# nju-websoft/MultiKE

Measured on AMD Instinct MI355X. Metric: scored triples/sec (pos+neg), higher is better.
Workload: dtype f32; 1 GPU; relation-view train step, C2-synth |E|=200000 |R|=550 dim=75 neg=25 batch=5000; n_ent=200000, n_rel=550, dim=75, neg=25, batch=5000, steps_per_epoch=184

## Files before the change

### include/multike_hip.h

```cpp
#ifndef MULTIKE_HIP_H
#define MULTIKE_HIP_H

#include <stdint.h>

#ifdef __cplusplus
extern "C" {
#endif

#define MKE_VERSION 106

#define MKE_OK 0
#define MKE_E_NULL (-1)
#define MKE_E_SHAPE (-2)
#define MKE_E_UNSUPPORTED (-3)
#define MKE_E_RANGE (-4)

#define MKE_LOSS_PARTIALS 2048

#define MKE_MAX_STRIDE 320

#define MKE_OPT_ADAGRAD 0
#define MKE_OPT_SGD 1
#define MKE_OPT_ADAM 2
#define MKE_OPT_ADADELTA 3

int mke_version(void);
const char* mke_last_error(void);

#define MKE_TUNE_DEFAULT (-2)
typedef struct mke_tuning {
  int score_splits, score_half_groups, score_offsets32, score_lane_ids, count_in_score, update_chunk, oc_score_quarter,
      attr_fused_bwd, sampler_fast;
  int reserved[7];
} mke_tuning;
int mke_tuning_init(mke_tuning* t);

int mke_set_option(const char* name, int value, int* old_value);


int mke_triple_score_fwd_bwd(
    const float* ent_table, int64_t n_ent, int ent_normalize,
    const float* rel_table, int64_t n_rel, int rel_normalize,
    int stride, int dim,
    const int32_t* pos_h, const int32_t* pos_r, const int32_t* pos_t, const float* pos_w ,
    int64_t n_pos,
    const int32_t* neg_h, const int32_t* neg_r, const int32_t* neg_t, const float* neg_w ,
    int64_t n_neg, int neg_per_pos,
    float scale,
    float* grad_ent , float* grad_rel , int grad_rel_copies,
    int32_t* touched_ent, int32_t* touched_rel, int32_t tag,
    double* loss_partials ,
    void* stream);

int mke_triple_score_fwd_bwd_det(
    float* ent_table, int64_t n_ent, int ent_normalize, const float* rel_table, int64_t n_rel, int rel_normalize,
    int stride, int dim, const int32_t* pos_h, const int32_t* pos_r, const int32_t* pos_t, const float* pos_w,
    int64_t n_pos, const int32_t* neg_h, const int32_t* neg_r, const int32_t* neg_t, const float* neg_w, int64_t n_neg,
    int neg_per_pos, float scale, float* grad_ent, float* grad_rel, int32_t* touched_ent, int32_t* touched_rel, int32_t tag,
    int32_t* ref_count , float* ent_acc, int optimizer, float lr, float* stage_rows, int64_t* stage_keys,
    int64_t stage_slots, double* loss_partials, void* stream);
int mke_stage_reduce(const float* stage_rows, const int64_t* sorted_keys, const int64_t* order, int64_t n_slots, int stride,
                     float* grad_ent, float* grad_rel, int32_t* touched_ent, int32_t* touched_rel, int32_t tag, void* stream);
int mke_count_entity_refs(const int32_t* pos_h, const int32_t* pos_t, int64_t n_pos, const int32_t* neg_h,
                          const int32_t* neg_t, int64_t n_neg, int neg_per_pos, int32_t* ref_count, void* stream);
int mke_triple_score_fwd_bwd_x(
    float* ent_table, int64_t n_ent, int ent_normalize,
    const float* rel_table, int64_t n_rel, int rel_normalize,
    int stride, int dim,
    const int32_t* pos_h, const int32_t* pos_r, const int32_t* pos_t, const float* pos_w , int64_t n_pos,
    const int32_t* neg_h, const int32_t* neg_r, const int32_t* neg_t, const float* neg_w , int64_t n_neg,
    int neg_per_pos, float scale,
    float* grad_ent, float* grad_rel, int grad_rel_copies,
    int32_t* touched_ent, int32_t* touched_rel, int32_t tag,
    int32_t* ref_count, float* ent_acc , int optimizer, float lr,
    double* loss_partials, void* stream);

struct mke_count_job;
typedef struct mke_hot_rows {
  const int32_t* slot;
  int32_t n_hot, copies;
  int64_t row0;
} mke_hot_rows;
int mke_triple_score_fwd_bwd_xc(
    float* ent_table, int64_t n_ent, int ent_normalize,
    const float* rel_table, int64_t n_rel, int rel_normalize,
    int stride, int dim,
// ... 454 lines not shown
```

### multike_amd/_lib.py

```python
from __future__ import annotations

import ctypes as C
import os

import numpy as np
import torch

_HERE = os.path.dirname(os.path.abspath(__file__))
SO_PATH = os.path.join(_HERE, "libmultike_hip.so")

LOSS_PARTIALS = 2048
MAX_STRIDE = 320
OPT_ADAGRAD, OPT_SGD, OPT_ADAM, OPT_ADADELTA = 0, 1, 2, 3
DENSE_OPTS = {"Adam": OPT_ADAM, "Adadelta": OPT_ADADELTA}
_SUPPORTED_FPL = (1, 2, 3, 4, 5, 6, 7, 8, 10, 12, 13, 16, 20)

SYMBOLS = (
    "mke_version", "mke_last_error", "mke_set_option", "mke_triple_score_fwd_bwd", "mke_triple_score_fwd_bwd_x",
    "mke_count_entity_refs", "mke_triple_score_fwd_bwd_xc", "mke_triple_score_fwd_bwd_xch", "mke_triple_score_fwd_bwd_det", "mke_stage_reduce", "mke_rows_update", "mke_rows_update_multi", "mke_rows_update_multi_count",
    "mke_neg_sample", "mke_tripleset_build", "mke_tripleset_query", "mke_gathered_logistic_fwd_bwd",
    "mke_gathered_alignment_fwd_bwd", "mke_align_fwd_bwd", "mke_gather_rows", "mke_relation_steps",
    "mke_rowset_build", "mke_rowset_remap", "mke_rows_gather_padded", "mke_rows_scatter_add",
    "mke_attr_conv_fwd", "mke_attr_conv_bwd", "mke_attr_tail_z", "mke_attr_tail_loss", "mke_attr_tail_bwd",
    "mke_dense_update", "mke_align_rank", "mke_gemm_f32", "mke_attr_scratch_floats", "mke_attr_step", "mke_attr_steps", "mke_attr_step_phases",
# ... 26 lines not shown
class AlignTableStruct(C.Structure):
    _fields_ = [("table", C.c_void_p), ("acc", C.c_void_p), ("grad", C.c_void_p), ("touched", C.c_void_p), ("n_rows", C.c_int64),
                ("normalize", C.c_int)]


class AlignTermStruct(C.Structure):
    _fields_ = [("a", C.c_int), ("b", C.c_int), ("weight", C.c_float)]


class AlignPlanStruct(C.Structure):
    _fields_ = [("tables", AlignTableStruct * 4), ("n_tables", C.c_int), ("terms", AlignTermStruct * 4), ("n_terms", C.c_int),
                ("stride", C.c_int), ("dim", C.c_int), ("ia", C.c_void_p), ("ib", C.c_void_p),
                ("step_off", C.POINTER(C.c_int64)), ("n_steps", C.c_int), ("optimizer", C.c_int), ("lr", C.c_float),
                ("tag_base", C.c_int32), ("loss_partials", C.c_void_p)]


class MappingViewStruct(C.Structure):
    _fields_ = [("table", C.c_void_p), ("normalize", C.c_int)]


class MappingStepArgs(C.Structure):
    _fields_ = [("ent_table", C.c_void_p), ("n_ent", C.c_int64), ("ent_normalize", C.c_int), ("ent_acc", C.c_void_p),
                ("ent_grad", C.c_void_p), ("ent_touched", C.c_void_p), ("views", MappingViewStruct * 3), ("n_views", C.c_int),
                ("stride", C.c_int), ("dim", C.c_int), ("idx", C.c_void_p), ("n", C.c_int64), ("M", C.c_void_p), ("gM", C.c_void_p),
                ("accM", C.c_void_p), ("orthogonal_weight", C.c_float), ("norm_w", C.c_float), ("scratch", C.c_void_p),
                ("partials", C.c_void_p), ("optimizer", C.c_int), ("lr", C.c_float), ("tag", C.c_int32), ("update", C.c_int)]


class HotRowsStruct(C.Structure):
    _fields_ = [("slot", C.c_void_p), ("n_hot", C.c_int32), ("copies", C.c_int32), ("row0", C.c_int64)]


class OcStepStruct(C.Structure):
    _fields_ = [("ent", C.c_void_p), ("ent_acc", C.c_void_p), ("ent_grad", C.c_void_p), ("ent_touched", C.c_void_p),
                ("ref_count", C.c_void_p), ("n_local", C.c_int64),
                ("rel", C.c_void_p), ("rel_acc", C.c_void_p), ("rel_grad", C.c_void_p), ("rel_grad_copies", C.c_int), ("rel_touched", C.c_void_p),
                ("n_rel", C.c_int64), ("stride", C.c_int), ("dim", C.c_int), ("rank", C.c_int), ("n_ranks", C.c_int),
                ("pos_h", C.c_void_p), ("pos_r", C.c_void_p), ("pos_t", C.c_void_p), ("n_pos", C.c_int64), ("per", C.c_int64),
                ("slot_h", C.c_void_p), ("slot_t", C.c_void_p), ("own_h", C.c_void_p), ("n_own_h", C.c_int64),
                ("own_t", C.c_void_p), ("n_own_t", C.c_int64), ("neg_per_pos", C.c_int), ("capacity", C.c_int64),
                ("codes", C.c_void_p), ("code_off", C.c_int64 * 16),
                ("optimizer", C.c_int), ("lr", C.c_float), ("scale", C.c_float), ("tag", C.c_int32),
                ("n_peers", C.c_int), ("peer_v", C.c_void_p * 16), ("peer_g", C.c_void_p * 16), ("pos_w", C.c_void_p),
                ("hot", HotRowsStruct),
                ("em_coef", C.c_void_p), ("em_pos0", C.c_int64), ("em_refs", C.c_void_p), ("em_rows", C.c_void_p), ("em_off", C.c_void_p),
                ("em_n_rows", C.c_int64), ("em_chunks", C.c_int), ("em_block_floats", C.c_int64), ("em_v", C.c_void_p * 4),
                ("em_gv", C.c_void_p * 4),
                ("em_part", C.c_void_p), ("em_long_rows", C.c_void_p), ("em_long_part0", C.c_void_p), ("em_n_long", C.c_int64),
                ("em_part0", C.c_int64), ("em_partials", C.c_void_p), ("em_mode", C.c_int), ("tuning", C.c_void_p)]


TUNE_DEFAULT = -2
TUNING_FIELDS = ("score_splits", "score_half_groups", "score_offsets32", "score_lane_ids", "count_in_score", "update_chunk",
                 "oc_score_quarter", "attr_fused_bwd", "sampler_fast")


class TuningStruct(C.Structure):
    _fields_ = [(f, C.c_int) for f in TUNING_FIELDS] + [("reserved", C.c_int * 7)]


def tuning(**knobs) -> TuningStruct:
    t = TuningStruct()
    _check(lib().mke_tuning_init(C.byref(t)), "mke_tuning_init")
    for k, v in knobs.items():
        if k not in TUNING_FIELDS:
            raise MultiKEHipError(f"unknown tuning knob {k!r}")
        setattr(t, k, int(v))
    return t


def tuning_ptr(t) -> int | None:
    return C.addressof(t) if t is not None else None


OC_EM_MAX_CHUNKS = 4
OC_EM_WAVES = 32768


class OcEmPlanArgs(C.Structure):
    _fields_ = [("pos_h", C.c_void_p), ("pos_r", C.c_void_p), ("pos_t", C.c_void_p), ("codes", C.c_void_p), ("neg_per_pos", C.c_int),
                ("slot_h", C.c_void_p), ("slot_t", C.c_void_p), ("step_lo", C.c_void_p), ("n_steps", C.c_int), ("chunks", C.c_int),
                ("n_all", C.c_int64), ("max_step", C.c_int64), ("n_ranks", C.c_int), ("rank", C.c_int), ("n_local", C.c_int64), ("n_rel", C.c_int64),
                ("keys", C.c_void_p), ("keys_alt", C.c_void_p), ("capacity", C.c_int64), ("vals_alt", C.c_void_p), ("scratch8", C.c_void_p), ("wave_scratch", C.c_void_p),
                ("refs", C.c_void_p), ("rows", C.c_void_p), ("off", C.c_void_p), ("flags", C.c_void_p), ("scan", C.c_void_p),
                ("step_row0", C.c_void_p), ("n_refs", C.c_void_p),
                ("item_row", C.c_void_p), ("item_off", C.c_void_p), ("item_part", C.c_void_p), ("long_row", C.c_void_p), ("long_part0", C.c_void_p),
                ("step_item0", C.c_void_p), ("step_long0", C.c_void_p), ("step_part0", C.c_void_p),
                ("temp", C.c_void_p), ("temp_bytes", C.c_int64)]


OC_COMM_NCCL, OC_COMM_CALLBACK, OC_COMM_LOOPBACK = 0, 1, 2
OC_CB_MOVE = C.CFUNCTYPE(C.c_int, C.c_void_p, C.c_void_p, C.c_void_p, C.c_int64, C.c_void_p)
OC_CB_REDUCE = C.CFUNCTYPE(C.c_int, C.c_void_p, C.c_void_p, C.c_int64, C.c_void_p)


class OcCommStruct(C.Structure):
    _fields_ = [("kind", C.c_int), ("ctx", C.c_void_p), ("all_gather", C.c_void_p), ("reduce_scatter", C.c_void_p), ("all_reduce", C.c_void_p),
                ("world", C.c_int), ("rank", C.c_int), ("wire_gbps", C.c_float), ("latency_us", C.c_float)]


class OcLoopStruct(C.Structure):
    _fields_ = [("parts", C.c_void_p), ("step_part0", C.c_void_p), ("n_steps", C.c_int), ("chunks", C.c_int),
                ("send", C.c_void_p * 4), ("v_all", C.c_void_p * 4), ("g_all", C.c_void_p * 4), ("gv", C.c_void_p * 4), ("block_floats", C.c_int64),
                ("loss_ring", C.c_void_p), ("loss_stride", C.c_int64), ("tag_base", C.c_int32), ("comm", C.c_void_p), ("comm_stream", C.c_void_p),
                ("overlap_rs", C.c_int)]


class AEPlanStruct(C.Structure):
    _fields_ = [("n_layers", C.c_int), ("dims", C.c_int * 5), ("act", C.c_int), ("normalize", C.c_int),
                ("params", C.c_void_p), ("grads", C.c_void_p), ("acc", C.c_void_p), ("n_params", C.c_int64),
                ("w_off", C.c_int64 * 8), ("b_off", C.c_int64 * 8), ("optimizer", C.c_int), ("lr", C.c_float),
# ... 852 lines not shown
```

### multike_amd/csrc/mke_api.hip

```cpp
#include <cstdarg>
#include <cstdio>
#include <cstring>

#include "mke_common.h"

namespace mke {

static thread_local char g_err[512] = "";

void set_error(const char* fmt, ...) {
  va_list ap;
  va_start(ap, fmt);
  vsnprintf(g_err, sizeof(g_err), fmt, ap);
  va_end(ap);
}

int check_launch(const char* what) {
  const hipError_t e = hipGetLastError();
  if (e != hipSuccess) {
    set_error("%s: launch failed: %s", what, hipGetErrorString(e));
    return (int)e;
  }
  return MKE_OK;
}

}

namespace mke {
int g_score_splits = 0;
int g_score_half_max = -1;
int g_score_o32 = 1;
int g_count_in_score = 1;
int g_score_lane_ids = 1;
int g_update_chunk = 0;
int g_deterministic = 0;
int g_sampler_fast = 1;
int g_attr_fused_bwd = 1;
int g_oc_em_keys64 = 0;
int g_oc_score_quarter = -1;
thread_local const mke_tuning* tl_tuning = nullptr;
}

extern "C" int mke_tuning_init(mke_tuning* t) {
  if (!t) { mke::set_error("mke_tuning_init: NULL"); return MKE_E_NULL; }
  int* f = reinterpret_cast<int*>(t);
  for (size_t i = 0; i < sizeof(mke_tuning) / sizeof(int); ++i) f[i] = MKE_TUNE_DEFAULT;
  return MKE_OK;
}

extern "C" int mke_set_option(const char* name, int value, int* old_value) {
  if (!name) { mke::set_error("mke_set_option: NULL name"); return MKE_E_NULL; }
  if (!strcmp(name, "score_splits")) {
    if (old_value) *old_value = mke::g_score_splits;
    mke::g_score_splits = value < 0 ? 0 : value;
    return MKE_OK;
  }
  if (!strcmp(name, "score_half_groups")) {
    if (old_value) *old_value = mke::g_score_half_max;
    mke::g_score_half_max = value < 0 ? -1 : (value > 64 ? 64 : value);
    return MKE_OK;
  }
  if (!strcmp(name, "score_offsets32")) {
    if (old_value) *old_value = mke::g_score_o32;
    mke::g_score_o32 = value != 0;
    return MKE_OK;
  }
  if (!strcmp(name, "count_in_score")) {
    if (old_value) *old_value = mke::g_count_in_score;
    mke::g_count_in_score = value != 0;
    return MKE_OK;
  }
  if (!strcmp(name, "score_lane_ids")) {
    if (old_value) *old_value = mke::g_score_lane_ids;
    mke::g_score_lane_ids = value != 0;
    return MKE_OK;
  }
  if (!strcmp(name, "update_chunk")) {
    if (old_value) *old_value = mke::g_update_chunk;
    mke::g_update_chunk = value == 16 ? 16 : (value == 64 ? 64 : 0);
    return MKE_OK;
  }
  if (!strcmp(name, "oc_score_quarter")) {
    if (old_value) *old_value = mke::g_oc_score_quarter;
    mke::g_oc_score_quarter = value < 0 ? -1 : (value != 0);
    return MKE_OK;
  }
  if (!strcmp(name, "attr_fused_bwd")) {
    if (old_value) *old_value = mke::g_attr_fused_bwd;
    mke::g_attr_fused_bwd = value != 0;
    return MKE_OK;
  }
  if (!strcmp(name, "sampler_fast")) {
    if (old_value) *old_value = mke::g_sampler_fast;
    mke::g_sampler_fast = value != 0;
    return MKE_OK;
  }
  if (!strcmp(name, "oc_em_keys64")) {
    if (old_value) *old_value = mke::g_oc_em_keys64;
    mke::g_oc_em_keys64 = value != 0;
    return MKE_OK;
  }
  if (!strcmp(name, "deterministic")) {
    if (old_value) *old_value = mke::g_deterministic;
    mke::g_deterministic = value != 0;
    return MKE_OK;
  }
  mke::set_error("mke_set_option: unknown option '%s'", name);
  return MKE_E_UNSUPPORTED;
}

extern "C" int mke_version(void) { return MKE_VERSION; }
extern "C" const char* mke_last_error(void) { return mke::g_err; }
```

### multike_amd/csrc/mke_common.h

```cpp
#pragma once
#include <hip/hip_runtime.h>
#include <stdint.h>

#include "../../include/multike_hip.h"

#define MKE_BLOCK 256
#define MKE_SUBS_PER_BLOCK (MKE_BLOCK / 16)
#define MKE_L2_EPS 1e-12f

namespace mke {

void set_error(const char* fmt, ...);
int check_launch(const char* what);

template <int CTRL>
__device__ __forceinline__ float dpp_mov(float v) {
  return __builtin_bit_cast(
      float, __builtin_amdgcn_update_dpp(0, __builtin_bit_cast(int, v), CTRL, 0xF, 0xF, true));
}

__device__ __forceinline__ float sub16_sum(float v) {
  v += dpp_mov<0xB1>(v);
  v += dpp_mov<0x4E>(v);
  v += dpp_mov<0x141>(v);
// ... 25 lines not shown
__device__ __forceinline__ void atomic_add_f32(float* p, float v) {
  __hip_atomic_fetch_add(p, v, __ATOMIC_RELAXED, __HIP_MEMORY_SCOPE_AGENT);
}

template <int FPL>
__device__ __forceinline__ void atomic_add_row(float* __restrict__ grad, int64_t row, int stride, int dim,
                                               int j, const float (&v)[FPL], float sgn) {
  float* p = grad + row * (int64_t)stride + j;
#pragma unroll
  for (int k = 0; k < FPL; ++k) {
    if (k * 16 + 16 <= dim || k * 16 + j < dim) atomic_add_f32(p + k * 16, sgn * v[k]);
  }
}

__device__ __forceinline__ float softplus_f(float x) {
  return fmaxf(x, 0.f) + __logf(1.0f + __expf(-fabsf(x)));
}
__device__ __forceinline__ float sigmoid_f(float x) { return __builtin_amdgcn_rcpf(1.0f + __expf(-x)); }
__device__ __forceinline__ float tanh_f(float x) {
  const float e = __expf(-2.0f * fabsf(x));
  return copysignf((1.0f - e) * __builtin_amdgcn_rcpf(1.0f + e), x);
}
__device__ __forceinline__ float adagrad_scale(float a) { return __builtin_amdgcn_rsqf(a); }

__device__ __forceinline__ void count_refs_range(const mke_count_job& c, int64_t block, int64_t n_blocks) {
  const int64_t total = c.n_pos + c.n_neg;
  for (int64_t i = block * MKE_BLOCK + threadIdx.x; i < total; i += n_blocks * MKE_BLOCK) {
    if (i < c.n_pos) {
      atomicAdd(&c.ref_count[c.pos_h[i]], 1);
      atomicAdd(&c.ref_count[c.pos_t[i]], 1);
    } else {
      const int64_t n = i - c.n_pos;
      const int64_t g = n / c.neg_per_pos;
      const int a = c.neg_h[n], b = c.neg_t[n];
      if (a != c.pos_h[g]) atomicAdd(&c.ref_count[a], 1);
      if (b != c.pos_t[g]) atomicAdd(&c.ref_count[b], 1);
    }
  }
}

extern thread_local int64_t g_update_touched_hint;
struct UpdateTouchedHint {
  explicit UpdateTouchedHint(int64_t rows) { g_update_touched_hint = rows; }
  ~UpdateTouchedHint() { g_update_touched_hint = 0; }
};

extern thread_local const mke_tuning* tl_tuning;
struct TuningScope {
  const mke_tuning* prev;
  explicit TuningScope(const mke_tuning* t) : prev(tl_tuning) { if (t) tl_tuning = t; }
  ~TuningScope() { tl_tuning = prev; }
};
extern int g_score_splits, g_score_half_max, g_score_o32, g_score_lane_ids, g_count_in_score, g_update_chunk, g_oc_score_quarter,
    g_attr_fused_bwd, g_sampler_fast;
#define MKE_TUNE(field, dflt) ((mke::tl_tuning && mke::tl_tuning->field != MKE_TUNE_DEFAULT) ? mke::tl_tuning->field : (dflt))
inline int tune_score_splits() { const int v = MKE_TUNE(score_splits, g_score_splits); return v < 0 ? 0 : v; }
inline int tune_score_half_max() { const int v = MKE_TUNE(score_half_groups, g_score_half_max); return v < 0 ? -1 : (v > 64 ? 64 : v); }
inline int tune_score_o32() { return MKE_TUNE(score_offsets32, g_score_o32) != 0; }
inline int tune_score_lane_ids() { return MKE_TUNE(score_lane_ids, g_score_lane_ids) != 0; }
inline int tune_count_in_score() { return MKE_TUNE(count_in_score, g_count_in_score) != 0; }
inline int tune_update_chunk() { const int v = MKE_TUNE(update_chunk, g_update_chunk); return v == 16 ? 16 : (v == 64 ? 64 : 0); }
inline int tune_oc_score_quarter() { const int v = MKE_TUNE(oc_score_quarter, g_oc_score_quarter); return v < 0 ? -1 : (v != 0); }
inline int tune_attr_fused_bwd() { return MKE_TUNE(attr_fused_bwd, g_attr_fused_bwd) != 0; }
inline int tune_sampler_fast() { return MKE_TUNE(sampler_fast, g_sampler_fast) != 0; }

__device__ __forceinline__ double block_sum_double(float v) {
  __shared__ double s_part[MKE_BLOCK / 64];
  double d = (double)v;
#pragma unroll
  for (int off = 32; off > 0; off >>= 1) d += __shfl_down(d, off, 64);
  const int wave = threadIdx.x >> 6;
  if ((threadIdx.x & 63) == 0) s_part[wave] = d;
  __syncthreads();
  double tot = 0.0;
  if (threadIdx.x == 0) {
#pragma unroll
    for (int w = 0; w < MKE_BLOCK / 64; ++w) tot += s_part[w];
  }
  return tot;
}

struct DenseJob {
  float* w;
  float* acc;
  float* g;
  int64_t n;
  int optimizer;
  float lr;
  float* ws;
  int ws_n, ws_stride, ws_copies;
};
__device__ __forceinline__ void dense_update_range(const DenseJob& j, int64_t block, int64_t n_blocks) {
  for (int64_t i = block * MKE_BLOCK + threadIdx.x; i < j.n; i += n_blocks * MKE_BLOCK) {
    float gv = j.g[i];
    if (j.ws && i < j.ws_n) {
#pragma unroll 8
      for (int c = 0; c < j.ws_copies; ++c) gv += j.ws[(size_t)c * j.ws_stride + i];
      for (int c = 0; c < j.ws_copies; ++c) j.ws[(size_t)c * j.ws_stride + i] = 0.f;
    }
    j.g[i] = 0.f;
    if (j.optimizer == MKE_OPT_ADAGRAD) {
      const float a = fmaf(gv, gv, j.acc[i]);
      j.acc[i] = a;
      j.w[i] -= j.lr * gv * adagrad_scale(a);
    } else {
      j.w[i] -= j.lr * gv;
    }
  }
}

struct Philox4 {
  uint32_t v[4];
};
__host__ __device__ __forceinline__ Philox4 philox4x32_10(uint32_t c0, uint32_t c1, uint32_t c2, uint32_t c3,
                                                          uint32_t k0, uint32_t k1) {
  const uint32_t M0 = 0xD2511F53u, M1 = 0xCD9E8D57u, W0 = 0x9E3779B9u, W1 = 0xBB67AE85u;
#pragma unroll
// ... 48 lines not shown
```

### multike_amd/csrc/mke_score.hip

```cpp
#include "mke_common.h"

namespace mke {

#ifndef MKE_SCORE_U
#define MKE_SCORE_U 2
#endif

struct ScoreParams {
  const float* ent;
  const float* __restrict__ rel;
  int ent_norm, rel_norm;
  int stride, dim;
  const int32_t* __restrict__ ph;
  const int32_t* __restrict__ pr;
  const int32_t* __restrict__ pt;
  const float* __restrict__ pw;
  int64_t n_pos;
  const int32_t* __restrict__ nh;
  const int32_t* __restrict__ nr;
  const int32_t* __restrict__ nt;
  const float* __restrict__ nw;
  int64_t n_neg;
  int npp;
  int splits;
  float scale;
  float* __restrict__ gent;
  float* __restrict__ grel;
  int grel_copies;
  int64_t grel_copy_elems;
  int32_t* __restrict__ tent;
  int32_t* __restrict__ trel;
  int32_t tag;
  double* __restrict__ lossp;
  int32_t* __restrict__ refcount;
  float* ent_w;
  float* __restrict__ ent_acc;
  int optimizer;
  float lr;
  float* __restrict__ stage_rows;
  int64_t* __restrict__ stage_keys;
  mke_count_job cj;
  int count_blocks;
  const int32_t* __restrict__ hot_slot;
  int32_t n_hot, hot_copies;
  int32_t hot_row0;
};

#define MKE_STAGE_REL (1ll << 40)
__device__ __forceinline__ int64_t stage_slot(int64_t g, int npp, int n, int c) { return ((g * (npp + 1) + n) * 3 + c); }

template <int FPL, bool O32>
__device__ __forceinline__ float* row_at(const float* base, int row, int stride, int j) {
  if (O32) return (float*)((char*)const_cast<float*>(base) + (((uint32_t)row * (uint32_t)(FPL * 16) + (uint32_t)j) << 2));
  return const_cast<float*>(base) + (int64_t)row * stride + j;
}
template <int FPL>
__device__ __forceinline__ void load_at(const float* __restrict__ q, float (&v)[FPL]) {
#pragma unroll
  for (int k = 0; k < FPL; ++k) v[k] = q[k * 16];
}
template <int FPL>
__device__ __forceinline__ void atomic_add_at(float* __restrict__ q, int dim, int j, const float (&v)[FPL], float sgn) {
#pragma unroll
  for (int k = 0; k < FPL; ++k) {
    if (k * 16 + 16 <= dim || k * 16 + j < dim) atomic_add_f32(q + k * 16, sgn * v[k]);
  }
}

template <int FPL, bool DET = false, bool O32 = false>
__device__ __forceinline__ void emit_row(const ScoreParams& p, bool is_rel, float* __restrict__ table_grad, int32_t* __restrict__ touched,
                                         int row, int64_t slot, int j, const float (&v)[FPL], float sgn, int grad_row = -1) {
  if (DET) {
    float* o = p.stage_rows + slot * p.stride + j;
#pragma unroll
    for (int k = 0; k < FPL; ++k) o[k * 16] = sgn * v[k];
    if (j == 0) p.stage_keys[slot] = (is_rel ? MKE_STAGE_REL : 0ll) | (int64_t)row;
  } else {
    atomic_add_at<FPL>(row_at<FPL, O32>(table_grad, grad_row >= 0 ? grad_row : row, p.stride, j), p.dim, j, v, sgn);
    if (j == 0) touched[row] = p.tag;
  }
}

template <bool DET>
__device__ __forceinline__ int hot_copy_row(const ScoreParams& p, int e, int64_t k) {
  if (DET || !p.hot_slot) return -1;
  const int s = p.hot_slot[e];
  return s >= 0 ? p.hot_row0 + (int)((uint32_t)k % (uint32_t)p.hot_copies) * p.n_hot + s : -1;
}

template <int FPL, bool DET = false>
__device__ __forceinline__ float independent_triple(const ScoreParams& p, float* __restrict__ grel, int j, int h, int r,
                                                    int t, float w, float sign, int64_t slot0) {
  float H[FPL], R[FPL], T[FPL];
  load_row<FPL>(p.ent, h, p.stride, j, H);
  load_row<FPL>(p.rel, r, p.stride, j, R);
  load_row<FPL>(p.ent, t, p.stride, j, T);
  l2_normalize_row<FPL>(H, p.ent_norm);
  l2_normalize_row<FPL>(R, p.rel_norm);
  l2_normalize_row<FPL>(T, p.ent_norm);
  float x = 0.f;
#pragma unroll
  for (int k = 0; k < FPL; ++k) {
    H[k] = (H[k] + R[k]) - T[k];
    x = fmaf(H[k], H[k], x);
  }
  x = sub16_sum(x);
  const float z = sign * x;
  const float l = w * softplus_f(z);
  if (p.gent) {
    const float c = 2.0f * sign * w * p.scale * sigmoid_f(z);
#pragma unroll
    for (int k = 0; k < FPL; ++k) H[k] *= c;
    emit_row<FPL, DET>(p, false, p.gent, p.tent, h, slot0, j, H, 1.0f, hot_copy_row<DET>(p, h, slot0 / 3));
    emit_row<FPL, DET>(p, true, grel, p.trel, r, slot0 + 1, j, H, 1.0f);
    emit_row<FPL, DET>(p, false, p.gent, p.tent, t, slot0 + 2, j, H, -1.0f, hot_copy_row<DET>(p, t, slot0 / 3));
  }
  return l;
}

template <int FPL, int U, bool X, int QPG, bool DET = false, bool O32 = false, bool LID = false>
__global__ __launch_bounds__(MKE_BLOCK) void k_triple_score(const ScoreParams p) {
  constexpr bool LIDS = LID && X && !DET;
  constexpr int LPG = 64 / (4 / QPG);
  if ((int)blockIdx.x < p.count_blocks) {
    count_refs_range(p.cj, blockIdx.x, p.count_blocks);
    if (threadIdx.x == 0) p.lossp[blockIdx.x] = 0.0;
    return;
  }
  const int bid = blockIdx.x - p.count_blocks, nblk = gridDim.x - p.count_blocks;
  const int lane = threadIdx.x & 63;
  const int j = lane & 15;
  const int q4 = lane >> 4;
  constexpr int GPW = 4 / QPG;
  const int sub = QPG == 4 ? 0 : (q4 >> 1);
  const int q = QPG == 4 ? q4 : (q4 & 1);
  const int64_t wave0 = ((int64_t)bid * MKE_BLOCK + threadIdx.x) >> 6;
  const int64_t nwaves = ((int64_t)nblk * MKE_BLOCK) >> 6;
  const bool bwd = p.gent != nullptr;
  float loss = 0.f;

  const int npp = p.npp;
  if (npp > 0) {
    const int S = QPG == 2 ? 1 : p.splits;
    const int64_t nitems = p.n_pos * S;
    const int64_t nwork = (nitems + GPW - 1) / GPW;
    for (int64_t wv = wave0; wv < nwork; wv += nwaves) {
      const int64_t wk_raw = wv * GPW + sub;
      const bool active = wk_raw < nitems;
      const int64_t wk = active ? wk_raw : 0;
      int64_t g;
      int s;
      if constexpr (QPG == 2) { g = wk; s = 0; }
      else { s = (int)((uint32_t)wk / (uint32_t)p.n_pos); g = (int64_t)((uint32_t)wk - (uint32_t)s * (uint32_t)p.n_pos); }
      float* __restrict__ grel = bwd ? p.grel + (int64_t)((uint32_t)wk % (uint32_t)p.grel_copies) * p.grel_copy_elems : nullptr;
      const int ph = p.ph[g], pr = p.pr[g], pt = p.pt[g];
      int hot_h = -1, hot_t = -1;
      if (!DET && p.hot_slot) {
        const int sh = p.hot_slot[ph], st = p.hot_slot[pt];
        const int cp = p.hot_row0 + (int)((uint32_t)g % (uint32_t)p.hot_copies) * p.n_hot;
        hot_h = sh >= 0 ? cp + sh : -1;
        hot_t = st >= 0 ? cp + st : -1;
      }
      const int npp_ = p.npp;
      const int per_ = (npp_ + S - 1) / S;
      const int nlo_ = s * per_, nend_ = min(npp_, nlo_ + per_);
      const int lbase = lane & ~(LPG - 1);
      int el = 0, fl = 0, rcl = 0, nblk = 0;
      float wl = 1.0f;
      bool slow_l = false;
      auto fetch_block = [&](int b0) {
        nblk = min(LPG, nend_ - b0);
        const bool has = active && lane - lbase < nblk;
        const int64_t idx = g * (int64_t)npp_ + (has ? b0 + (lane - lbase) : 0);
        const int nh = p.nh[idx], nr = p.nr[idx], nt = p.nt[idx];
        wl = p.nw ? p.nw[idx] : 1.0f;
        const bool dh = nh != ph, dt = nt != pt;
        const bool fastl = has && (nr == pr) && (dh != dt);
        el = dh ? nh : nt;
        fl = (fastl ? 1 : 0) | (dh ? 2 : 0);
        slow_l = has && !fastl;
        rcl = fastl ? p.refcount[el] : 0;
      };
      if constexpr (LIDS) fetch_block(nlo_);
      float H[FPL], R[FPL], T[FPL];
      load_at<FPL>(row_at<FPL, O32>(p.ent, ph, p.stride, j), H);
      load_at<FPL>(row_at<FPL, O32>(p.rel, pr, p.stride, j), R);
      load_at<FPL>(row_at<FPL, O32>(p.ent, pt, p.stride, j), T);
      l2_normalize_row<FPL>(H, p.ent_norm);
      l2_normalize_row<FPL>(R, p.rel_norm);
      l2_normalize_row<FPL>(T, p.ent_norm);
      float gH[FPL], gT[FPL];
      float gP[FPL];
      float HR[FPL], RT[FPL];
#pragma unroll
      for (int k = 0; k < FPL; ++k) {
        gH[k] = gT[k] = gP[k] = 0.f;
        HR[k] = H[k] + R[k];
        RT[k] = R[k] - T[k];
      }

      if (s == 0 && q == 0 && active) {
        const float w = p.pw ? p.pw[g] : 1.0f;
        float d[FPL];
        float x = 0.f;
#pragma unroll
        for (int k = 0; k < FPL; ++k) {
          d[k] = HR[k] - T[k];
          x = fmaf(d[k], d[k], x);
        }
        x = sub16_sum(x);
        loss += w * softplus_f(x);
        const float c = 2.0f * w * p.scale * sigmoid_f(x);
#pragma unroll
        for (int k = 0; k < FPL; ++k) {
          const float gd = c * d[k];
          gH[k] += gd; gT[k] += gd; gP[k] = gd;
        }
      }

      const int per = (npp + S - 1) / S;
      const int n_lo = s * per;
      const int n_hi = active ? min(npp, n_lo + per) : n_lo;
      const int64_t nbase = g * (int64_t)npp;
      bool any_slow = false;
      const int n_end = min(npp, n_lo + per);
      for (int b0 = n_lo; b0 < (LIDS ? n_end : n_lo + 1); b0 += LPG) {
      if constexpr (LIDS) {
        if (b0 != n_lo) fetch_block(b0);
        any_slow |= __any(slow_l) != 0;
      }
      const int it_lo = LIDS ? 0 : n_lo + q, it_hi = LIDS ? nblk : n_hi, it_step = QPG * U;
      for (int n0 = it_lo; n0 < it_hi; n0 += it_step) {
        int e[U], cnt[U];
        bool fast[U], sideH[U];
        float w[U];
        float C[U][FPL];
        float A[X ? U : 1][X ? FPL : 1];
#pragma unroll
        for (int u = 0; u < U; ++u) {
          if constexpr (LIDS) {
            const int slot = n0 + q + QPG * u;
            const bool live = slot < nblk;
            const int src = lbase + (live ? slot : 0);
            e[u] = __shfl(el, src, 64);
            const int f = __shfl(fl, src, 64);
            cnt[u] = __shfl(rcl, src, 64);
            w[u] = __shfl(wl, src, 64);
            fast[u] = live && (f & 1);
            sideH[u] = (f & 2) != 0;
          } else {
            const int n = n0 + QPG * u;
            const bool live = n < n_hi;
            const int64_t idx = nbase + (live ? n : n_lo);
            const int nh = p.nh[idx], nr = p.nr[idx], nt = p.nt[idx];
            w[u] = p.nw ? p.nw[idx] : 1.0f;
            const bool dh = nh != ph, dt = nt != pt;
            fast[u] = live && (nr == pr) && (dh != dt);
            sideH[u] = dh;
            e[u] = dh ? nh : nt;
            any_slow |= live && !fast[u];
          }
        }
#pragma unroll
        for (int u = 0; u < U; ++u) {
          if constexpr (!LIDS) cnt[u] = 0;
          if (fast[u]) {
            load_at<FPL>(row_at<FPL, O32>(p.ent, e[u], p.stride, j), C[u]);
            if constexpr (X) {
              if constexpr (!LIDS) cnt[u] = p.refcount[e[u]];
              if (p.ent_acc && (!LIDS || cnt[u] == 1)) load_at<FPL>(row_at<FPL, O32>(p.ent_acc, e[u], p.stride, j), A[u]);
            }
          }
        }
#pragma unroll
        for (int u = 0; u < U; ++u) {
          if (fast[u]) {
            float cinv = 1.0f;
            if (p.ent_norm) {
              float ss = 0.f;
#pragma unroll
              for (int k = 0; k < FPL; ++k) ss = fmaf(C[u][k], C[u][k], ss);
              cinv = rsqrtf(fmaxf(sub16_sum(ss), MKE_L2_EPS));
            }
            float d[FPL];
            float y = 0.f;
            const float sc = sideH[u] ? cinv : -cinv;
#pragma unroll
            for (int k = 0; k < FPL; ++k) {
              d[k] = fmaf(sc, C[u][k], sideH[u] ? RT[k] : HR[k]);
              y = fmaf(d[k], d[k], y);
            }
            y = sub16_sum(y);
            const float t_ = __expf(-y);
            const float s1 = 1.0f + t_;
            loss += w[u] * __logf(s1);
            if (bwd) {
              const float c = -2.0f * w[u] * p.scale * t_ * __builtin_amdgcn_rcpf(s1);
              const float cH = sideH[u] ? 0.f : c;
              const float cT = sideH[u] ? c : 0.f;
#pragma unroll
              for (int k = 0; k < FPL; ++k) {
                gH[k] = fmaf(cH, d[k], gH[k]);
                gT[k] = fmaf(cT, d[k], gT[k]);
                d[k] *= c;
              }
              bool in_place = false;
              if constexpr (X) in_place = cnt[u] == 1;
              if (in_place) {
                const float sg = sideH[u] ? 1.0f : -1.0f;
                float g[FPL];
                if (p.ent_norm) {
                  float dot = 0.f;
#pragma unroll
                  for (int k = 0; k < FPL; ++k) dot = fmaf(C[u][k], d[k], dot);
                  dot = sub16_sum(dot) * (sg * cinv);
                  const float a1 = sg * cinv;
                  const float a2 = cinv < 0.99e6f ? -dot * cinv * cinv : 0.f;
#pragma unroll
                  for (int k = 0; k < FPL; ++k) g[k] = fmaf(a2, C[u][k], a1 * d[k]);
                } else {
#pragma unroll
                  for (int k = 0; k < FPL; ++k) g[k] = sg * d[k];
                }
                float* wp = row_at<FPL, O32>(p.ent_w, e[u], p.stride, j);
                if (p.optimizer == MKE_OPT_ADAGRAD) {
                  float* ap = row_at<FPL, O32>(p.ent_acc, e[u], p.stride, j);
#pragma unroll
                  for (int k = 0; k < FPL; ++k) {
                    const float a = fmaf(g[k], g[k], A[u][k]);
                    ap[k * 16] = a;
                    wp[k * 16] = C[u][k] - p.lr * g[k] * adagrad_scale(a);
                  }
                } else {
#pragma unroll
                  for (int k = 0; k < FPL; ++k) wp[k * 16] = C[u][k] - p.lr * g[k];
                }
                if (j == 0) p.refcount[e[u]] = 0;
              } else {
                emit_row<FPL, DET, O32>(p, false, p.gent, p.tent, e[u], stage_slot(g, npp, n0 + QPG * u, sideH[u] ? 0 : 2), j, d,
                              sideH[u] ? 1.0f : -1.0f);
              }
            }
          }
        }
      }
      }

      if (any_slow) {
#pragma unroll 1
        for (int n = n_lo + q; n < n_hi; n += QPG) {
          const int64_t idx = nbase + n;
          const int nh = p.nh[idx], nr = p.nr[idx], nt = p.nt[idx];
          if (!((nr == pr) && ((nh != ph) != (nt != pt))))
            loss += independent_triple<FPL, DET>(p, grel, j, nh, nr, nt, p.nw ? p.nw[idx] : 1.0f, -1.0f, stage_slot(g, npp, n, 0));
        }
      }

      if (bwd) {
        float gR[FPL];
#pragma unroll
        for (int k = 0; k < FPL; ++k) {
          gR[k] = (gH[k] + gT[k]) - gP[k];
          gH[k] += __shfl_xor(gH[k], 16, 64);
          gR[k] += __shfl_xor(gR[k], 16, 64);
          gT[k] += __shfl_xor(gT[k], 16, 64);
          if (QPG == 4) {
            gH[k] += __shfl_xor(gH[k], 32, 64);
            gR[k] += __shfl_xor(gR[k], 32, 64);
            gT[k] += __shfl_xor(gT[k], 32, 64);
          }
        }
        if (active && (s == 0 || n_lo < n_hi)) {
          if (QPG == 4) {
            float v[FPL];
#pragma unroll
            for (int k = 0; k < FPL; ++k) v[k] = q == 0 ? gH[k] : (q == 1 ? gR[k] : -gT[k]);
            float* __restrict__ base = q == 1 ? grel : p.gent;
            const int row = q == 0 ? ph : (q == 1 ? pr : pt);
            if (q < 3) emit_row<FPL, DET>(p, q == 1, base, q == 1 ? p.trel : p.tent, row, stage_slot(g, npp, npp, q), j, v, 1.0f,
                                          q == 0 ? hot_h : (q == 2 ? hot_t : -1));
          } else {
            float v[FPL];
#pragma unroll
            for (int k = 0; k < FPL; ++k) v[k] = q == 0 ? gH[k] : -gT[k];
            const int row = q == 0 ? ph : pt;
            emit_row<FPL, DET>(p, false, p.gent, p.tent, row, stage_slot(g, npp, npp, q == 0 ? 0 : 2), j, v, 1.0f, q == 0 ? hot_h : hot_t);
            if (q == 0) emit_row<FPL, DET>(p, true, grel, p.trel, pr, stage_slot(g, npp, npp, 1), j, gR, 1.0f);
          }
        }
      }
    }
  } else {
    const int64_t sub0 = ((int64_t)bid * MKE_BLOCK + threadIdx.x) >> 4;
    const int64_t nsub = ((int64_t)nblk * MKE_BLOCK) >> 4;
    for (int64_t i = sub0; i < p.n_pos + p.n_neg; i += nsub) {
      float* __restrict__ grel = bwd ? p.grel + (int64_t)((uint32_t)i % (uint32_t)p.grel_copies) * p.grel_copy_elems : nullptr;
      if (i < p.n_pos) {
        loss += independent_triple<FPL, DET>(p, grel, j, p.ph[i], p.pr[i], p.pt[i], p.pw ? p.pw[i] : 1.0f, 1.0f, i * 3);
      } else {
        const int64_t n = i - p.n_pos;
        loss += independent_triple<FPL, DET>(p, grel, j, p.nh[n], p.nr[n], p.nt[n], p.nw ? p.nw[n] : 1.0f, -1.0f, i * 3);
      }
    }
  }

  const double tot = block_sum_double(j == 0 ? loss : 0.f);
  if (threadIdx.x == 0) p.lossp[blockIdx.x] = tot * (double)p.scale;
}

__global__ __launch_bounds__(MKE_BLOCK) void k_count_refs(const int32_t* __restrict__ ph, const int32_t* __restrict__ pt,
                                                          int64_t n_pos, const int32_t* __restrict__ nh,
                                                          const int32_t* __restrict__ nt, int64_t n_neg, int npp,
                                                          int32_t* __restrict__ cnt) {
  const int64_t total = n_pos + n_neg;
  for (int64_t i = (int64_t)blockIdx.x * MKE_BLOCK + threadIdx.x; i < total; i += (int64_t)gridDim.x * MKE_BLOCK) {
    if (i < n_pos) {
      atomicAdd(&cnt[ph[i]], 1);
      atomicAdd(&cnt[pt[i]], 1);
    } else {
      const int64_t n = i - n_pos;
      const int64_t g = n / npp;
      const int a = nh[n], b = nt[n];
      if (a != ph[g]) atomicAdd(&cnt[a], 1);
      if (b != pt[g]) atomicAdd(&cnt[b], 1);
    }
  }
}

}

static int score_impl(
    const float* ent_table, int64_t n_ent, int ent_normalize, const float* rel_table, int64_t n_rel,
    int rel_normalize, int stride, int dim, const int32_t* pos_h, const int32_t* pos_r, const int32_t* pos_t,
    const float* pos_w, int64_t n_pos, const int32_t* neg_h, const int32_t* neg_r, const int32_t* neg_t,
    const float* neg_w, int64_t n_neg, int neg_per_pos, float scale, float* grad_ent, float* grad_rel,
    int grad_rel_copies, int32_t* touched_ent, int32_t* touched_rel, int32_t tag, double* loss_partials, void* stream,
    int32_t* ref_count, float* ent_w, float* ent_acc, int optimizer, float lr, float* stage_rows = nullptr,
    int64_t* stage_keys = nullptr, int64_t stage_slots = 0, const mke_count_job* next_count = nullptr,
    const mke_hot_rows* hot = nullptr) {
// ... 13 lines not shown
  }
  if ((grad_ent == nullptr) != (grad_rel == nullptr)) { set_error("grad_ent and grad_rel must both be given or both NULL"); return MKE_E_NULL; }
  if (grad_ent && (!touched_ent || !touched_rel)) { set_error("NULL touched array"); return MKE_E_NULL; }
  if (grad_ent && (grad_rel_copies < 1 || grad_rel_copies > 64)) { set_error("grad_rel_copies must be in [1,64]"); return MKE_E_SHAPE; }

  ScoreParams p;
  p.ent = ent_table; p.rel = rel_table; p.ent_norm = ent_normalize; p.rel_norm = rel_normalize;
  p.stride = stride; p.dim = dim;
  p.ph = pos_h; p.pr = pos_r; p.pt = pos_t; p.pw = pos_w; p.n_pos = n_pos;
  p.nh = neg_h; p.nr = neg_r; p.nt = neg_t; p.nw = neg_w; p.n_neg = n_neg;
  p.npp = neg_per_pos;
  const int64_t total_waves = (int64_t)MKE_LOSS_PARTIALS * (MKE_BLOCK / 64);
  int splits = 1;
  if (neg_per_pos > 0 && n_pos > 0) {
    int64_t s = total_waves / n_pos;
    const int64_t smax = (neg_per_pos + 3) / 4;
    if (s > smax) s = smax;
    if (s < 1) s = 1;
    if (tune_score_splits() > 0) s = tune_score_splits();
    if (s > neg_per_pos) s = neg_per_pos;
    splits = (int)s;
  }
  if (stage_keys) {
    splits = 1;
    const int64_t need = (neg_per_pos > 0 ? n_pos * (neg_per_pos + 1) : n_pos + n_neg) * 3;
    if (!stage_rows || !grad_ent || need > stage_slots) { set_error("deterministic mode: %lld staging slots needed, %lld given", (long long)need, (long long)stage_slots); return MKE_E_SHAPE; }
  }
  p.stage_rows = stage_rows; p.stage_keys = stage_keys;
  p.hot_slot = nullptr; p.n_hot = 0; p.hot_copies = 1; p.hot_row0 = 0;
  if (hot && hot->slot && hot->n_hot > 0 && grad_ent && !stage_keys) {
    if (hot->copies < 1 || hot->row0 < n_ent || (hot->row0 + (int64_t)hot->copies * hot->n_hot) * stride >= (1ll << 31)) {
      set_error("hub rows: copies >= 1, row0 >= n_ent and the copy rows inside 2^31 floats of the scratch");
      return MKE_E_SHAPE;
    }
    p.hot_slot = hot->slot; p.n_hot = hot->n_hot; p.hot_copies = hot->copies; p.hot_row0 = (int32_t)hot->row0;
  }
  p.cj = mke_count_job{};
  p.count_blocks = 0;
  if (next_count && next_count->n_pos + next_count->n_neg > 0) {
    if (!next_count->ref_count || !next_count->pos_h || !next_count->pos_t || (next_count->n_neg > 0 && (!next_count->neg_h || !next_count->neg_t))) { set_error("count job: NULL pointer"); return MKE_E_NULL; }
    int64_t cb = (next_count->n_pos + next_count->n_neg + 4 * MKE_BLOCK - 1) / (4 * MKE_BLOCK);
    p.cj = *next_count;
    if (p.cj.neg_per_pos < 1) p.cj.neg_per_pos = 1;
    p.count_blocks = (int)std::min<int64_t>(cb, MKE_LOSS_PARTIALS / 4);
  }
  p.splits = splits;
  p.scale = scale;
  p.gent = grad_ent; p.grel = grad_rel; p.grel_copies = grad_rel_copies < 1 ? 1 : grad_rel_copies;
  p.grel_copy_elems = n_rel * (int64_t)stride;
  p.tent = touched_ent; p.trel = touched_rel; p.tag = tag;
  p.lossp = loss_partials;
  const bool excl = ref_count != nullptr && grad_ent != nullptr && neg_per_pos > 0;
  p.refcount = excl ? ref_count : nullptr; p.ent_w = ent_w; p.ent_acc = ent_acc; p.optimizer = optimizer; p.lr = lr;
  hipStream_t st = (hipStream_t)stream;
  const int fpl = stride / 16;
  const int64_t grad_rows = p.hot_slot ? (int64_t)p.hot_row0 + (int64_t)p.hot_copies * p.n_hot : n_ent;
  const bool o32 = tune_score_o32() && grad_rows * (int64_t)stride < (1ll << 30) && n_rel * (int64_t)stride < (1ll << 30);
  MKE_DISPATCH_FPL(fpl, {
    constexpr int U = FPL <= 5 ? MKE_SCORE_U : (FPL <= 8 ? 2 : 1);
    const int half_max = tune_score_half_max() >= 0 ? tune_score_half_max() : (FPL <= 8 ? 64 : 31);
    const bool half = neg_per_pos > 0 && neg_per_pos <= half_max && splits == 1;
    if (n_pos * (int64_t)splits > 0xFFFFFFFFll || n_pos + n_neg > 0xFFFFFFFFll) { set_error("more than 2^32 work items in one launch"); return MKE_E_RANGE; }
    if (stage_keys) {
      if (half) {
        if (excl) hipLaunchKernelGGL((k_triple_score<FPL, U, true, 2, true>), dim3(MKE_LOSS_PARTIALS), dim3(MKE_BLOCK), 0, st, p);
        else hipLaunchKernelGGL((k_triple_score<FPL, U, false, 2, true>), dim3(MKE_LOSS_PARTIALS), dim3(MKE_BLOCK), 0, st, p);
      } else {
        if (excl) hipLaunchKernelGGL((k_triple_score<FPL, U, true, 4, true>), dim3(MKE_LOSS_PARTIALS), dim3(MKE_BLOCK), 0, st, p);
        else hipLaunchKernelGGL((k_triple_score<FPL, U, false, 4, true>), dim3(MKE_LOSS_PARTIALS), dim3(MKE_BLOCK), 0, st, p);
      }
    } else if (excl && o32) {
      if (half && tune_score_lane_ids()) hipLaunchKernelGGL((k_triple_score<FPL, U, true, 2, false, true, true>), dim3(MKE_LOSS_PARTIALS), dim3(MKE_BLOCK), 0, st, p);
      else if (half) hipLaunchKernelGGL((k_triple_score<FPL, U, true, 2, false, true>), dim3(MKE_LOSS_PARTIALS), dim3(MKE_BLOCK), 0, st, p);
      else if (tune_score_lane_ids()) hipLaunchKernelGGL((k_triple_score<FPL, U, true, 4, false, true, true>), dim3(MKE_LOSS_PARTIALS), dim3(MKE_BLOCK), 0, st, p);
      else hipLaunchKernelGGL((k_triple_score<FPL, U, true, 4, false, true>), dim3(MKE_LOSS_PARTIALS), dim3(MKE_BLOCK), 0, st, p);
    } else if (half) {
      if (excl) hipLaunchKernelGGL((k_triple_score<FPL, U, true, 2>), dim3(MKE_LOSS_PARTIALS), dim3(MKE_BLOCK), 0, st, p);
      else hipLaunchKernelGGL((k_triple_score<FPL, U, false, 2>), dim3(MKE_LOSS_PARTIALS), dim3(MKE_BLOCK), 0, st, p);
    } else {
      if (excl) hipLaunchKernelGGL((k_triple_score<FPL, U, true, 4>), dim3(MKE_LOSS_PARTIALS), dim3(MKE_BLOCK), 0, st, p);
      else hipLaunchKernelGGL((k_triple_score<FPL, U, false, 4>), dim3(MKE_LOSS_PARTIALS), dim3(MKE_BLOCK), 0, st, p);
    }
  });
  return check_launch("k_triple_score");
}

extern "C" int mke_triple_score_fwd_bwd(
    const float* ent_table, int64_t n_ent, int ent_normalize, const float* rel_table, int64_t n_rel,
    int rel_normalize, int stride, int dim, const int32_t* pos_h, const int32_t* pos_r, const int32_t* pos_t,
    const float* pos_w, int64_t n_pos, const int32_t* neg_h, const int32_t* neg_r, const int32_t* neg_t,
    const float* neg_w, int64_t n_neg, int neg_per_pos, float scale, float* grad_ent, float* grad_rel,
    int grad_rel_copies, int32_t* touched_ent, int32_t* touched_rel, int32_t tag, double* loss_partials, void* stream) {
  return score_impl(ent_table, n_ent, ent_normalize, rel_table, n_rel, rel_normalize, stride, dim, pos_h, pos_r, pos_t, pos_w,
                    n_pos, neg_h, neg_r, neg_t, neg_w, n_neg, neg_per_pos, scale, grad_ent, grad_rel, grad_rel_copies,
                    touched_ent, touched_rel, tag, loss_partials, stream, nullptr, nullptr, nullptr, 0, 0.f);
}

extern "C" int mke_triple_score_fwd_bwd_xc(
    float* ent_table, int64_t n_ent, int ent_normalize, const float* rel_table, int64_t n_rel, int rel_normalize,
    int stride, int dim, const int32_t* pos_h, const int32_t* pos_r, const int32_t* pos_t, const float* pos_w,
    int64_t n_pos, const int32_t* neg_h, const int32_t* neg_r, const int32_t* neg_t, const float* neg_w, int64_t n_neg,
    int neg_per_pos, float scale, float* grad_ent, float* grad_rel, int grad_rel_copies, int32_t* touched_ent,
    int32_t* touched_rel, int32_t tag, int32_t* ref_count, float* ent_acc, int optimizer, float lr,
    const mke_count_job* next_count, double* loss_partials, void* stream) {
  using namespace mke;
  if (optimizer != MKE_OPT_ADAGRAD && optimizer != MKE_OPT_SGD) { set_error("unsupported optimizer %d", optimizer); return MKE_E_UNSUPPORTED; }
// ... 135 lines not shown
```

Before: 2.383 billion triples/s.

## Apply optimizer in place for positive head/tail rows owned exclusively by one triple

Extends the existing exclusive-row in-place update, which was used only for negative-sample rows, to the positive head/tail entity rows. When the refcount shows the row is referenced once, it is not hot-replicated, and no lane in the group took the slow path, the kernel reloads the weight and accumulator, applies the norm-aware gradient and the Adagrad or SGD step directly, and clears the refcount. This skips the atomic gradient scatter and the later row-update pass for those rows. The in-place math is factored into a shared helper. The cost is extra refcount and weight loads, a ballot, and more branching, and the result depends on the refcount being exact.

```diff
diff --git a/include/multike_hip.h b/include/multike_hip.h
--- a/include/multike_hip.h
+++ b/include/multike_hip.h
@@ -30,8 +30,8 @@
 #define MKE_TUNE_DEFAULT (-2)
 typedef struct mke_tuning {
   int score_splits, score_half_groups, score_offsets32, score_lane_ids, count_in_score, update_chunk, oc_score_quarter,
-      attr_fused_bwd, sampler_fast;
-  int reserved[7];
+      attr_fused_bwd, sampler_fast, score_flush_inplace;
+  int reserved[6];
 } mke_tuning;
 int mke_tuning_init(mke_tuning* t);
 
diff --git a/multike_amd/_lib.py b/multike_amd/_lib.py
--- a/multike_amd/_lib.py
+++ b/multike_amd/_lib.py
@@ -102,11 +102,11 @@
 
 TUNE_DEFAULT = -2
 TUNING_FIELDS = ("score_splits", "score_half_groups", "score_offsets32", "score_lane_ids", "count_in_score", "update_chunk",
-                 "oc_score_quarter", "attr_fused_bwd", "sampler_fast")
+                 "oc_score_quarter", "attr_fused_bwd", "sampler_fast", "score_flush_inplace")
 
 
 class TuningStruct(C.Structure):
-    _fields_ = [(f, C.c_int) for f in TUNING_FIELDS] + [("reserved", C.c_int * 7)]
+    _fields_ = [(f, C.c_int) for f in TUNING_FIELDS] + [("reserved", C.c_int * 6)]
 
 
 def tuning(**knobs) -> TuningStruct:
diff --git a/multike_amd/csrc/mke_api.hip b/multike_amd/csrc/mke_api.hip
--- a/multike_amd/csrc/mke_api.hip
+++ b/multike_amd/csrc/mke_api.hip
@@ -32,6 +32,7 @@
 int g_score_o32 = 1;
 int g_count_in_score = 1;
 int g_score_lane_ids = 1;
+int g_score_flush_inplace = 1;
 int g_update_chunk = 0;
 int g_deterministic = 0;
 int g_sampler_fast = 1;
@@ -75,6 +76,11 @@
     mke::g_score_lane_ids = value != 0;
     return MKE_OK;
   }
+  if (!strcmp(name, "score_flush_inplace")) {
+    if (old_value) *old_value = mke::g_score_flush_inplace;
+    mke::g_score_flush_inplace = value != 0;
+    return MKE_OK;
+  }
   if (!strcmp(name, "update_chunk")) {
     if (old_value) *old_value = mke::g_update_chunk;
     mke::g_update_chunk = value == 16 ? 16 : (value == 64 ? 64 : 0);
diff --git a/multike_amd/csrc/mke_common.h b/multike_amd/csrc/mke_common.h
--- a/multike_amd/csrc/mke_common.h
+++ b/multike_amd/csrc/mke_common.h
@@ -101,7 +101,7 @@
   ~TuningScope() { tl_tuning = prev; }
 };
 extern int g_score_splits, g_score_half_max, g_score_o32, g_score_lane_ids, g_count_in_score, g_update_chunk, g_oc_score_quarter,
-    g_attr_fused_bwd, g_sampler_fast;
+    g_attr_fused_bwd, g_sampler_fast, g_score_flush_inplace;
 #define MKE_TUNE(field, dflt) ((mke::tl_tuning && mke::tl_tuning->field != MKE_TUNE_DEFAULT) ? mke::tl_tuning->field : (dflt))
 inline int tune_score_splits() { const int v = MKE_TUNE(score_splits, g_score_splits); return v < 0 ? 0 : v; }
 inline int tune_score_half_max() { const int v = MKE_TUNE(score_half_groups, g_score_half_max); return v < 0 ? -1 : (v > 64 ? 64 : v); }
@@ -112,6 +112,7 @@
 inline int tune_oc_score_quarter() { const int v = MKE_TUNE(oc_score_quarter, g_oc_score_quarter); return v < 0 ? -1 : (v != 0); }
 inline int tune_attr_fused_bwd() { return MKE_TUNE(attr_fused_bwd, g_attr_fused_bwd) != 0; }
 inline int tune_sampler_fast() { return MKE_TUNE(sampler_fast, g_sampler_fast) != 0; }
+inline int tune_score_flush_inplace() { return MKE_TUNE(score_flush_inplace, g_score_flush_inplace) != 0; }
 
 __device__ __forceinline__ double block_sum_double(float v) {
   __shared__ double s_part[MKE_BLOCK / 64];
diff --git a/multike_amd/csrc/mke_score.hip b/multike_amd/csrc/mke_score.hip
--- a/multike_amd/csrc/mke_score.hip
+++ b/multike_amd/csrc/mke_score.hip
@@ -44,6 +44,7 @@
   const int32_t* __restrict__ hot_slot;
   int32_t n_hot, hot_copies;
   int32_t hot_row0;
+  int32_t flush_inplace;
 };
 
 #define MKE_STAGE_REL (1ll << 40)
@@ -79,6 +80,39 @@
     atomic_add_at<FPL>(row_at<FPL, O32>(table_grad, grad_row >= 0 ? grad_row : row, p.stride, j), p.dim, j, v, sgn);
     if (j == 0) touched[row] = p.tag;
   }
+}
+
+template <int FPL, bool O32>
+__device__ __forceinline__ void finish_row_in_place(const ScoreParams& p, int row, int j, const float (&W)[FPL], const float (&A)[FPL],
+                                                    const float (&gn)[FPL], float sg, float cinv) {
+  float g[FPL];
+  if (p.ent_norm) {
+    float dot = 0.f;
+#pragma unroll
+    for (int k = 0; k < FPL; ++k) dot = fmaf(W[k], gn[k], dot);
+    dot = sub16_sum(dot) * (sg * cinv);
+    const float a1 = sg * cinv;
+    const float a2 = cinv < 0.99e6f ? -dot * cinv * cinv : 0.f;
+#pragma unroll
+    for (int k = 0; k < FPL; ++k) g[k] = fmaf(a2, W[k], a1 * gn[k]);
+  } else {
+#pragma unroll
+    for (int k = 0; k < FPL; ++k) g[k] = sg * gn[k];
+  }
+  float* wp = row_at<FPL, O32>(p.ent_w, row, p.stride, j);
+  if (p.optimizer == MKE_OPT_ADAGRAD) {
+    float* ap = row_at<FPL, O32>(p.ent_acc, row, p.stride, j);
+#pragma unroll
+    for (int k = 0; k < FPL; ++k) {
+      const float a = fmaf(g[k], g[k], A[k]);
+      ap[k * 16] = a;
+      wp[k * 16] = W[k] - p.lr * g[k] * adagrad_scale(a);
+    }
+  } else {
+#pragma unroll
+    for (int k = 0; k < FPL; ++k) wp[k * 16] = W[k] - p.lr * g[k];
+  }
+  if (j == 0) p.refcount[row] = 0;
 }
 
 template <bool DET>
@@ -160,6 +194,10 @@
         const int cp = p.hot_row0 + (int)((uint32_t)g % (uint32_t)p.hot_copies) * p.n_hot;
         hot_h = sh >= 0 ? cp + sh : -1;
         hot_t = st >= 0 ? cp + st : -1;
+      }
+      int rc_own = 0;
+      if constexpr (X && !DET) {
+        if (p.flush_inplace) rc_own = p.refcount[q == 0 ? ph : pt];
       }
       const int npp_ = p.npp;
       const int per_ = (npp_ + S - 1) / S;
@@ -223,11 +261,13 @@
       const int n_hi = active ? min(npp, n_lo + per) : n_lo;
       const int64_t nbase = g * (int64_t)npp;
       bool any_slow = false;
+      uint64_t slow_bits = 0;
       const int n_end = min(npp, n_lo + per);
       for (int b0 = n_lo; b0 < (LIDS ? n_end : n_lo + 1); b0 += LPG) {
       if constexpr (LIDS) {
         if (b0 != n_lo) fetch_block(b0);
-        any_slow |= __any(slow_l) != 0;
+        slow_bits |= __ballot(slow_l);
+        any_slow = slow_bits != 0;
       }
       const int it_lo = LIDS ? 0 : n_lo + q, it_hi = LIDS ? nblk : n_hi, it_step = QPG * U;
       for (int n0 = it_lo; n0 < it_hi; n0 += it_step) {
@@ -307,35 +347,7 @@
               bool in_place = false;
               if constexpr (X) in_place = cnt[u] == 1;
               if (in_place) {
-                const float sg = sideH[u] ? 1.0f : -1.0f;
-                float g[FPL];
-                if (p.ent_norm) {
-                  float dot = 0.f;
-#pragma unroll
-                  for (int k = 0; k < FPL; ++k) dot = fmaf(C[u][k], d[k], dot);
-                  dot = sub16_sum(dot) * (sg * cinv);
-                  const float a1 = sg * cinv;
-                  const float a2 = cinv < 0.99e6f ? -dot * cinv * cinv : 0.f;
-#pragma unroll
-                  for (int k = 0; k < FPL; ++k) g[k] = fmaf(a2, C[u][k], a1 * d[k]);
-                } else {
-#pragma unroll
-                  for (int k = 0; k < FPL; ++k) g[k] = sg * d[k];
-                }
-                float* wp = row_at<FPL, O32>(p.ent_w, e[u], p.stride, j);
-                if (p.optimizer == MKE_OPT_ADAGRAD) {
-                  float* ap = row_at<FPL, O32>(p.ent_acc, e[u], p.stride, j);
-#pragma unroll
-                  for (int k = 0; k < FPL; ++k) {
-                    const float a = fmaf(g[k], g[k], A[u][k]);
-                    ap[k * 16] = a;
-                    wp[k * 16] = C[u][k] - p.lr * g[k] * adagrad_scale(a);
-                  }
-                } else {
-#pragma unroll
-                  for (int k = 0; k < FPL; ++k) wp[k * 16] = C[u][k] - p.lr * g[k];
-                }
-                if (j == 0) p.refcount[e[u]] = 0;
+                if constexpr (X) finish_row_in_place<FPL, O32>(p, e[u], j, C[u], A[u], d, sideH[u] ? 1.0f : -1.0f, cinv);
               } else {
                 emit_row<FPL, DET, O32>(p, false, p.gent, p.tent, e[u], stage_slot(g, npp, n0 + QPG * u, sideH[u] ? 0 : 2), j, d,
                               sideH[u] ? 1.0f : -1.0f);
@@ -370,6 +382,27 @@
             gT[k] += __shfl_xor(gT[k], 32, 64);
           }
         }
+        bool fin = false;
+        if constexpr (X && !DET) {
+          const uint64_t gm = LPG == 64 ? ~0ull : (0xFFFFFFFFull << lbase);
+          const uint64_t sb = LIDS ? slow_bits : __ballot(any_slow);
+          fin = (QPG == 4 ? (q == 0 || q == 2) : true) && rc_own == 1 && (q == 0 ? hot_h : hot_t) < 0 && (sb & gm) == 0;
+        }
+        auto finish_own = [&](int row, const float (&v)[FPL]) {
+          if constexpr (X && !DET) {
+            float W[FPL], A[FPL];
+            load_at<FPL>(row_at<FPL, O32>(p.ent, row, p.stride, j), W);
+            if (p.ent_acc) load_at<FPL>(row_at<FPL, O32>(p.ent_acc, row, p.stride, j), A);
+            float cinv = 1.0f;
+            if (p.ent_norm) {
+              float ss = 0.f;
+#pragma unroll
+              for (int k = 0; k < FPL; ++k) ss = fmaf(W[k], W[k], ss);
+              cinv = rsqrtf(fmaxf(sub16_sum(ss), MKE_L2_EPS));
+            }
+            finish_row_in_place<FPL, O32>(p, row, j, W, A, v, 1.0f, cinv);
+          }
+        };
         if (active && (s == 0 || n_lo < n_hi)) {
           if (QPG == 4) {
             float v[FPL];
@@ -377,14 +410,16 @@
             for (int k = 0; k < FPL; ++k) v[k] = q == 0 ? gH[k] : (q == 1 ? gR[k] : -gT[k]);
             float* __restrict__ base = q == 1 ? grel : p.gent;
             const int row = q == 0 ? ph : (q == 1 ? pr : pt);
-            if (q < 3) emit_row<FPL, DET>(p, q == 1, base, q == 1 ? p.trel : p.tent, row, stage_slot(g, npp, npp, q), j, v, 1.0f,
-                                          q == 0 ? hot_h : (q == 2 ? hot_t : -1));
+            if (fin) finish_own(row, v);
+            else if (q < 3) emit_row<FPL, DET>(p, q == 1, base, q == 1 ? p.trel : p.tent, row, stage_slot(g, npp, npp, q), j, v, 1.0f,
+                                               q == 0 ? hot_h : (q == 2 ? hot_t : -1));
           } else {
             float v[FPL];
 #pragma unroll
             for (int k = 0; k < FPL; ++k) v[k] = q == 0 ? gH[k] : -gT[k];
             const int row = q == 0 ? ph : pt;
-            emit_row<FPL, DET>(p, false, p.gent, p.tent, row, stage_slot(g, npp, npp, q == 0 ? 0 : 2), j, v, 1.0f, q == 0 ? hot_h : hot_t);
+            if (fin) finish_own(row, v);
+            else emit_row<FPL, DET>(p, false, p.gent, p.tent, row, stage_slot(g, npp, npp, q == 0 ? 0 : 2), j, v, 1.0f, q == 0 ? hot_h : hot_t);
             if (q == 0) emit_row<FPL, DET>(p, true, grel, p.trel, pr, stage_slot(g, npp, npp, 1), j, gR, 1.0f);
           }
         }
@@ -504,6 +539,7 @@
   p.lossp = loss_partials;
   const bool excl = ref_count != nullptr && grad_ent != nullptr && neg_per_pos > 0;
   p.refcount = excl ? ref_count : nullptr; p.ent_w = ent_w; p.ent_acc = ent_acc; p.optimizer = optimizer; p.lr = lr;
+  p.flush_inplace = excl && !stage_keys && splits == 1 && !p.hot_slot && tune_score_flush_inplace();
   hipStream_t st = (hipStream_t)stream;
   const int fpl = stride / 16;
   const int64_t grad_rows = p.hot_slot ? (int64_t)p.hot_row0 + (int64_t)p.hot_copies * p.n_hot : n_ent;
```

Measured after the change: 2.423 billion triples/s (median of 6 runs). 1.02x the previous value.
